# csyxwei/FFWM

Measured on AMD Instinct MI355X. Metric: train img/s (128x128, full FFWM GAN step), higher is better.
Workload: dtype f32; 1 GPU; BASELINE configs[2]: full FFWM train step (netG+netD+flowNetF+flowNetB, all losses, 3x Adam), synthetic MultiPIE-shaped 128x128; batch_per_gpu=8, global_batch=8, parallelism=dp1, grad_buckets=10, bucket_MiB=64

## Files before the change

ffwm_amd/_lib.py:

```python
import ctypes
import os

_HERE = os.path.dirname(os.path.abspath(__file__))
LIB_PATH = os.path.join(_HERE, "lib", "libffwm_hip.so")

F32, F64 = 0, 1
ABI_VERSION = 5

_lib = None

_p = ctypes.c_void_p
_i64 = ctypes.c_int64
_i = ctypes.c_int

_SIGNATURES = {
    "ffwm_block_extractor_forward": [_p, _p, _p] + [_i64] * 6 + [_i, _i, _p],
    "ffwm_block_extractor_backward": [_p, _p, _p, _p, _p] + [_i64] * 6 + [_i, _i, _p],
    "ffwm_block_extractor_backward_strided": [_p, _p, _p, ctypes.POINTER(_i64), _p, _p] + [_i64] * 6 + [_i, _i, _p],
    "ffwm_local_attn_reshape_backward_strided": [_p, ctypes.POINTER(_i64), _p] + [_i64] * 3 + [_i, _i, _i, _p],
    "ffwm_resample2d_backward_strided": [_p, _p, _p, ctypes.POINTER(_i64), _p, _p] + [_i64] * 6 + [_i, _i, _i, _i, _p],
    "ffwm_bn_lrelu_forward": [_p] * 9 + [_i64] * 3 + [ctypes.c_double] * 3 + [_i, _p],
    "ffwm_bn_lrelu_backward": [_p] * 10 + [_i64] * 3 + [ctypes.c_double] + [_i, _p],
    "ffwm_bn_res_act_forward": [_p] * 11 + [_i64] * 3 + [ctypes.c_double] * 3 + [_i, _i, _p],
    "ffwm_bn_res_act_backward": [_p] * 11 + [_i64] * 3 + [ctypes.c_double] + [_i, _i, _p],
    "ffwm_mfm_forward": [_p, _p, _p] + [_i64] * 3 + [_i, _p],
    "ffwm_mfm_backward": [_p, _p, _p, _p] + [_i64] * 3 + [_i, _p],
    "ffwm_add_act_forward": [_p, _p, _p, _i64, _i, ctypes.c_double, _i, _p],
    "ffwm_add_act_backward": [_p, _p, _p, _i64, _i, ctypes.c_double, _i, _p],
    "ffwm_sigmoid_gate_forward": [_p, _p, _p, _p, _p, _i64, _i, _p],
    "ffwm_sigmoid_gate_backward": [_p, _p, _p, _p, _p, _i64, _i, _p],
    "ffwm_bias_relu_forward": [_p, _p, _p] + [_i64] * 3 + [_i, _p],
    "ffwm_bias_act_forward": [_p, _p, _p, _p] + [_i64] * 5 + [_i, ctypes.c_double, _i, _p],
    "ffwm_flow_head_forward": [_p, _p, _p, _p] + [_i64] * 4 + [_i, _p],
    "ffwm_conv_thin_forward": [_p, _p, _p, _p] + [_i64] * 5 + [_i, ctypes.c_double, _i, _p],
    "ffwm_flow_up_forward": [_p, _p, _p, _p] + [_i64] * 4 + [_i, _p],
    "ffwm_shuffle_bias_act_forward": [_p, _p, _p] + [_i64] * 5 + [ctypes.c_double, _i, _p],
    "ffwm_image_head_forward": [_p, _p, _p, _p] + [_i64] * 5 + [_i, _p],
    "ffwm_upsample2x_bilinear_forward": [_p, _p] + [_i64] * 5 + [_i, _p],
    "ffwm_sigmoid_gate_forward_strided": [_p, _p, _p, _p, _p] + [_i64] * 4 + [_i, _p],
    "ffwm_flow_head_backward": [_p, _p, _p, _p, _p] + [_i64] * 4 + [_i, _p],
    "ffwm_flow_up_backward": [_p, _p, _p] + [_i64] * 4 + [_i, _p],
    "ffwm_conv2d_forward": [_p, _p, _p, _p, _p] + [_i64] * 5 + [_i, _i, _i, _i, _i64, _i64, _i, ctypes.c_double, _p, _i64, _i, _p],
    "ffwm_conv2d_wgrad": [_p, _p, _p] + [_i64] * 7 + [_i, _i, _i, _i, _p],
    "ffwm_conv2d_wgrad_tiled": [_p, _p, _p, _p] + [_i64] * 7 + [_i, _i, _i, _i, _i, _p],
    "ffwm_conv3x3_winograd_forward": [_p, _p, _p, _p, _p] + [_i64] * 5 + [_i, _i, ctypes.c_double, _i, _p],
    "ffwm_adam_step": [_p, _p, _p, _p, _i64] + [ctypes.c_double] * 4 + [_i64, _i, _p],
    "ffwm_adam_step_device": [_p, _p, _p, _p, _i64] + [ctypes.c_double] * 4 + [_p, _i, _p],
    "ffwm_sgd_step": [_p, _p, _p, _i64, _p, _p, _i, _p, _p, _i, ctypes.c_double, _i, _p],
    "ffwm_softmax_xent": [_p] * 8 + [_i64, _i64, _i, _p],
    "ffwm_softmax_xent_chunk": [],
    "ffwm_conv3x3_wgrad": [_p, _p, _p, _p] + [_i64] * 5 + [_i, _p],
    "ffwm_conv3x3_wgrad_block": [_p, _p, _p, _p] + [_i64] * 9 + [_i, _p],
    "ffwm_block_attention_forward": [_p, _p, _p, _p] + [_i64] * 6 + [_i, _i, _p],
    "ffwm_block_attention_backward": [_p, _p, _p, _p, _p, _p, _p] + [_i64] * 6 + [_i, _i, _p],
    "ffwm_local_attn_reshape_forward": [_p, _p] + [_i64] * 3 + [_i, _i, _p],
    "ffwm_local_attn_reshape_backward": [_p, _p] + [_i64] * 3 + [_i, _i, _i, _p],
    "ffwm_resample2d_forward": [_p, _p, _p] + [_i64] * 6 + [_i, _i, _i, _p],
    "ffwm_resample2d_backward": [_p, _p, _p, _p, _p] + [_i64] * 6 + [_i, _i, _i, _i, _p],
    "ffwm_warp_forward": [_p, _p, _p] + [_i64] * 6 + [_i, _i, _p],
    "ffwm_warp_backward": [_p, _p, _p, _p, _p] + [_i64] * 6 + [_i, _i, _p],
    "ffwm_warp_multi_forward": [_p, _i, _i, _i, _p],
    "ffwm_warp_multi_backward": [_p, _i, _i, _i, _p],
    "ffwm_spectral_norm_forward": [_p, _i, _i, ctypes.c_double, _i, _p],
    "ffwm_spectral_norm_backward": [_p, _i, _i, _p],
    "ffwm_guided_filter_forward": [_p, _p, _p, _p, _i64, _i64, _i64, _i, ctypes.c_double, _i, _p],
    "ffwm_affine_regularization": [_p, _p, _p, _p, _i64, _i64, _i64, _i, ctypes.c_double, _i, _p],
    "ffwm_correlation_colmax": [_p, _p, _p, _i64, _i64, _i64, _i, _p],
    "ffwm_correlation_colmax_split": [_p, _p, _p, _i64, _i64, _i64, _i, _p],
    "ffwm_sampling_correctness": [_p] * 9 + [_i64] * 6 + [ctypes.c_double, ctypes.c_double, _i, _p],
    "ffwm_landmark_loss": [_p, _p, ctypes.POINTER(_i64), ctypes.POINTER(_i64), ctypes.POINTER(ctypes.c_double), _i] + [_p] * 6
                          + [_i64, _i64, _i, _p],
    "ffwm_guided_filter_backward": [_p, _p, _p, _p, _p, _p, _i64, _i64, _i64, _i, _i, _p],
    "ffwm_guided_filter_forward_general": [_p, _p, _p, _p, _p, _i64, _i64, _i64, _i64, _i, ctypes.c_double, _i, _p],
    "ffwm_guided_filter_backward_general": [_p, _p, _p, _p, _p, _p, _p, _i64, _i64, _i64, _i64, _i, _i, _p],
    "ffwm_l1_multi": [_p, _i, _p, _p, _i, _i, _p],
    "ffwm_conv3x3_winograd_weights_multi": [_p, _i, _i, _p],
    "ffwm_conv3x3_wg_weights": [_p, _p, _i64, _i64, _i, _i, _p],
    "ffwm_conv3x3_wg_forward": [_p, _p, _p, _p, _p] + [_i64] * 5 + [_i, _p, _i, _p],
    "ffwm_conv3x3_wg_forward_tiled": [_p, _p, _p, _p, _p] + [_i64] * 5 + [_i, _p, _i, _i, _p],
    "ffwm_conv3x3_wg_tile": [_i64] * 5,
    "ffwm_mfm_tail_forward": [_p, _p, _p, _p] + [_i64] * 4 + [_i, _i, _p],
    "ffwm_identity_input": [_p, _p] + [_i64] * 4 + [_i, _i, _p],
    "ffwm_identity_input_backward": [_p, _p] + [_i64] * 4 + [_i, _i, _p],
    "ffwm_cosine_topk": [_p, _p, _p, _p] + [_i64] * 4 + [_p, _i64, _i, _p],
    "ffwm_face_batch": [_p] * 16 + [_i64] * 8 + [_i, _p],
    "ffwm_face_gallery": [_p, _p, _p] + [_i64] * 4 + [_p],
    "ffwm_identity_batch": [_p] * 8 + [_i64] * 5 + [_i, _i, _p],
    "ffwm_prof_enable": [_i],
    "ffwm_prof_collect": [],
    "ffwm_prof_get": [_i, ctypes.c_char_p, _i, ctypes.POINTER(_i64), ctypes.POINTER(ctypes.c_double),
                      ctypes.POINTER(ctypes.c_double)],
    "ffwm_prof_get_flops": [_i, ctypes.POINTER(ctypes.c_double)],
    "ffwm_prof_get_bound": [_i, ctypes.POINTER(ctypes.c_double)],
    "ffwm_prof_reset": [],
    "ffwm_set_option": [ctypes.c_char_p, _i],
    "ffwm_zero_fill": [_p, _i64, _p],
    "ffwm_abi_version": [],
}

EXPORTS = sorted(list(_SIGNATURES) + ["ffwm_last_error", "ffwm_conv3x3_winograd_workspace_bytes", "ffwm_conv3x3_winograd_splits",
                                      "ffwm_conv2d_forward_workspace", "ffwm_guided_filter_workspace_bytes",
                                      "ffwm_sampling_correctness_workspace_bytes", "ffwm_landmark_loss_workspace_bytes",
                                      "ffwm_cosine_topk_workspace_bytes", "ffwm_softmax_xent_workspace_bytes",
                                      "ffwm_conv3x3_wg_weights_bytes", "ffwm_conv3x3_wg_workspace_bytes"])


class FFWMError(RuntimeError):
    pass


def load():
    global _lib
    if _lib is not None:
        return _lib
    if not os.path.exists(LIB_PATH):
        raise FFWMError(
            "libffwm_hip.so is missing (%s). The HIP extension is the only implementation of the "
            "ffwm_amd ops -- build it with `python -m ffwm_amd.build`." % LIB_PATH)
    lib = ctypes.CDLL(LIB_PATH)
    for name, argtypes in _SIGNATURES.items():
        fn = getattr(lib, name)
        fn.argtypes = argtypes
        fn.restype = _i
    lib.ffwm_conv3x3_winograd_workspace_bytes.argtypes = [_i64, _i64]
    lib.ffwm_conv3x3_winograd_workspace_bytes.restype = _i64
    lib.ffwm_conv3x3_winograd_splits.argtypes = [_i64, _i64, _i64, _i64, _i64, _i]
    lib.ffwm_conv3x3_winograd_splits.restype = _i
# ... 71 lines not shown
```

ffwm_amd/conv.py:

```python
import os as _os

import torch
import torch.nn as nn
from torch.autograd import Function

from . import ops

_WGRAD_W64 = _os.environ.get("FFWM_WGRAD_W64", "1") == "1"


class _Conv3x3MfmaWgrad(Function):

    @staticmethod
    def forward(ctx, x, weight, bias):
        ctx.save_for_backward(x, weight)
        ctx.has_bias = bias is not None
        return torch.ops.aten.convolution(x, weight, bias, [1, 1], [1, 1], [1, 1], False, [0, 0], 1)

    @staticmethod
    @torch.autograd.function.once_differentiable
    def backward(ctx, grad_output):
        x, weight = ctx.saved_tensors
        go = grad_output.contiguous()
        need_x, need_w, need_b = ctx.needs_input_grad[0], ctx.needs_input_grad[1], ctx.has_bias and ctx.needs_input_grad[2]
# ... 27 lines not shown
                and input.is_cuda and input.dtype == torch.float32 and not torch.is_autocast_enabled()):
            return _MfmaConv2d.apply(input, weight, bias, self.stride[0], self.padding[0], False)
        return super()._conv_forward(input, weight, bias)


def _tiled_wgrad_layer_ok(m):
    if m.kernel_size == (1, 1):
        return (_TILED_WGRAD and _TILED_WGRAD_1X1 and m.stride == (1, 1) and m.padding == (0, 0) and m.dilation == (1, 1) and m.groups == 1
                and min(m.in_channels, m.out_channels) >= 32)
    return (_TILED_WGRAD and m.kernel_size in ((3, 3), (4, 4)) and m.stride in ((1, 1), (2, 2)) and m.padding[0] == m.padding[1]
            and m.padding[0] < m.kernel_size[0] and m.dilation == (1, 1) and m.groups == 1 and m.padding_mode == "zeros")


def eligible(m):
    return (type(m) is nn.Conv2d and m.kernel_size == (3, 3) and m.stride == (1, 1) and m.padding == (1, 1)
            and m.dilation == (1, 1) and m.groups == 1 and m.padding_mode == "zeros"
            and (min(m.in_channels, m.out_channels) >= 64
                 or (min(m.in_channels, m.out_channels) <= 3 and max(m.in_channels, m.out_channels) >= 64)))


def route_conv_wgrad(net):
    n = 0
    for m in net.modules():
        if eligible(m):
            m.__class__ = MfmaWgradConv2d
            n += 1
    return n


_TILED_WGRAD = _os.environ.get("FFWM_TILED_WGRAD", "1") != "0"
_TILED_WGRAD_1X1 = _os.environ.get("FFWM_TILED_WGRAD_1X1", "1") != "0"


def _tiled_wgrad_wins(rows, gathered, kernel):
    K, P = rows.shape[1], rows.shape[2] * rows.shape[3]
    if not (_TILED_WGRAD and kernel in (1, 3, 4) and ops.conv2d_wgrad_tiled_ok(rows) and gathered.numel() < (1 << 29)):
        return False
    if kernel == 1 and (min(K, gathered.shape[1]) < 32 or not _TILED_WGRAD_1X1):
        return False
    if K <= 4 and (P >= 16384 or (P >= 4096 and gathered.shape[1] >= 128)):
        return False
    return True


class _GradArena:

    def __init__(self):
        self.buf, self.off, self.need, self.active, self.retired = None, 0, 0, False, []

    def begin(self, device):
        self.off = self.need = 0
        if self.buf is not None and self.buf.device != device:
            self.retired.append(self.buf)
            self.buf = None
        if self.buf is not None:
            ops.zero_fill(self.buf)
        self.active = True
        self.device = device

    def take(self, n, like):
        if not self.active or like.device != self.device or like.dtype != torch.float32:
            return None
        n_al = (n + 63) & ~63
        self.need += n_al
        if self.buf is None or self.off + n_al > self.buf.numel():
            return None
        s = self.buf[self.off:self.off + n]
        self.off += n_al
        return s

    def end(self):
        if not self.active:
            return
        self.active = False
        if (self.buf is None or self.need > self.buf.numel()) and self.need > 0 and not torch.cuda.is_current_stream_capturing():
            if self.buf is not None:
                self.retired.append(self.buf)
            self.buf = torch.zeros(self.need + self.need // 8, device=self.device, dtype=torch.float32)


GRAD_ARENA = _GradArena()


def conv_weight_grad(x, go, weight, stride, pad, need_b):
    k = weight.shape[2]
    if k == 3 and stride == 1 and pad == 1 and wgrad_route_ok(x, weight):
        n = weight.numel()
        total = n + (weight.shape[0] if need_b else 0)
        buf = GRAD_ARENA.take(total, go)
        if buf is None:
            buf = torch.zeros(total, device=go.device, dtype=go.dtype)
        gw, gb = buf[:n].view_as(weight), (buf[n:] if need_b else None)
        ops.conv3x3_wgrad(x, go, gw, gb)
        return gw, gb
    if _tiled_wgrad_wins(go, x, k) and weight.shape[2] == weight.shape[3]:
        return ops.conv2d_wgrad_tiled(go, x, k, stride, pad, want_bias=bool(need_b),
                                      zeroed=GRAD_ARENA.take(weight.numel() + (weight.shape[0] if need_b else 0), go))
    _, gw, gb = torch.ops.aten.convolution_backward(go, x, weight, [weight.shape[0]] if need_b else None, [stride, stride], [pad, pad],
                                                    [1, 1], False, [0, 0], 1, [False, True, bool(need_b)])
    return gw, gb


def conv_transpose_weight_grad(x, go, weight, need_b):
    if _tiled_wgrad_wins(x, go, 4):
        gw, _ = ops.conv2d_wgrad_tiled(x, go, 4, 2, 1, zeroed=GRAD_ARENA.take(weight.numel(), go))
        return gw, (_bias_grad(go) if need_b else None)
    _, gw, gb = torch.ops.aten.convolution_backward(go, x, weight, [weight.shape[1]] if need_b else None, [2, 2], [1, 1], [1, 1], True,
                                                    [0, 0], 1, [False, True, bool(need_b)])
    return gw, gb


_WINOGRAD = _os.environ.get("FFWM_WINOGRAD", "1") != "0"
WINOGRAD_MIN_TILES = int(_os.environ.get("FFWM_WINOGRAD_MIN_TILES", 2048))
WINOGRAD_MIN_PAIRS = int(_os.environ.get("FFWM_WINOGRAD_MIN_PAIRS", 160))


def _winograd_dir_ok(x, c_red, k_out, act=0):
    tiles = x.shape[0] * ((x.shape[2] + 1) // 2) * ((x.shape[3] + 1) // 2)
    if not (min(c_red, k_out) >= 32 and tiles >= WINOGRAD_MIN_TILES and x.shape[0] * max(c_red, k_out) * x.shape[2] * x.shape[3] < (1 << 29)):
        return False
    pairs = ((tiles + 63) // 64) * ((k_out + 63) // 64)
    if pairs < WINOGRAD_MIN_PAIRS and act == 0:
        pairs *= ops.conv3x3_winograd_splits(x.shape[0], c_red, x.shape[2], x.shape[3], k_out, act)
    return pairs >= WINOGRAD_MIN_PAIRS


def winograd_dirs(x, weight, act=0):
    if not (_WINOGRAD and x.is_cuda and x.dtype == torch.float32 and weight.dtype == torch.float32 and x.dim() == 4
            and not torch.is_autocast_enabled()):
        return False, False
    K, C = weight.shape[0], weight.shape[1]
    if K <= 4 and C >= 32:
        return x.shape[3] % 4 == 0 and x.shape[0] * x.shape[2] * x.shape[3] >= 65536 and x.numel() < (1 << 29), False
    return _winograd_dir_ok(x, C, K, act), _winograd_dir_ok(x, K, C)


def winograd_ok(x, weight, act=0):
    return winograd_dirs(x, weight, act)[0]


_WINO_BATCH = _os.environ.get("FFWM_WINO_BATCH", "1") != "0"


def _note_winograd_use(weight, x, dirs, need_dgrad):
    owner = getattr(weight, "_ffwm_wino_owner", None)
    if owner is None or not _WINO_BATCH:
        return None
    keys = owner.__dict__.setdefault("_wino_keys", set())
    wm4 = x.shape[3] % 4 == 0
    if dirs[0]:
        keys.add((0, wm4))
    if dirs[1] and need_dgrad:
        keys.add((1, wm4))
    return getattr(weight, "_ffwm_wino", None)


class _WinogradConv3x3(Function):

    @staticmethod
    def forward(ctx, x, weight, bias, frozen=None, dirs=(True, True)):
        pre = _note_winograd_use(weight, x, dirs, ctx.needs_input_grad[0])
        x, weight = x.contiguous(), weight.contiguous()
        ctx.save_for_backward(x, weight)
        ctx.has_bias = bias is not None
        ctx.frozen = frozen
        ctx.own_dgrad = dirs[1]
        ctx.wino_pre = pre
        if dirs[0]:
            return ops.conv3x3_winograd(x, weight, bias, frozen=frozen, pre=pre)
        return torch.ops.aten.convolution(x, weight, bias, [1, 1], [1, 1], [1, 1], False, [0, 0], 1)

    @staticmethod
    @torch.autograd.function.once_differentiable
    def backward(ctx, grad_output):
        x, weight = ctx.saved_tensors
        go = grad_output.contiguous()
        need_x, need_w, need_b = ctx.needs_input_grad[0], ctx.needs_input_grad[1], ctx.has_bias and ctx.needs_input_grad[2]
        gx = gw = gb = None
        if need_x and ctx.own_dgrad:
            gx = ops.conv3x3_winograd(go, weight, None, data_gradient=True, frozen=ctx.frozen, pre=ctx.wino_pre)
        elif need_x:
            gx = torch.ops.aten.convolution_backward(go, x, weight, None, [1, 1], [1, 1], [1, 1], False, [0, 0], 1, [True, False, False])[0]
        if need_w:
            gw, gb = conv_weight_grad(x, go, weight, 1, 1, need_b)
        if need_b and gb is None:
            gb = _bias_grad(go)
# ... 485 lines not shown
```

ffwm_amd/ops.py:

```python
import ctypes

import torch

from . import _lib

_DT = {torch.float32: _lib.F32, torch.float64: _lib.F64}


def _dtype_code(t):
    try:
        return _DT[t.dtype]
    except KeyError:
        raise TypeError("ffwm_amd ops support float32/float64 (AT_DISPATCH_FLOATING_TYPES), got %s" % t.dtype)


def _go_strides(grad_output):
    if grad_output.is_contiguous():
        return grad_output, None
    st = grad_output.stride()
    if any(x < 0 for x in st) or st[3] == 0:
        return grad_output.contiguous(), None
    return grad_output, (ctypes.c_int64 * 4)(*st)


# ... 559 lines not shown
                                         _ptr(ws), B, N, code, stream), "ffwm_softmax_xent")
    return out, row_loss, rank, grad, skipped


def conv3x3_wgrad_supported(input, grad_output):
    return (input.dtype == torch.float32 and grad_output.dtype == torch.float32 and input.is_cuda
            and input.shape[3] % 64 == 0 and input.numel() * 4 < (1 << 32) - 64 and grad_output.numel() * 4 < (1 << 32) - 64)


def conv3x3_wgrad(input, grad_output, grad_weight=None, grad_bias=None):
    _check("conv3x3_wgrad", input, grad_output, grad_weight)
    if grad_bias is not None and not (grad_bias.is_cuda and grad_bias.device == input.device and grad_bias.dtype == input.dtype
                                      and grad_bias.is_contiguous()):
        raise ValueError("conv3x3_wgrad: grad_bias must be a contiguous tensor on the input's device, same dtype")
    B, C, H, W = input.shape
    Bg, K, Hg, Wg = grad_output.shape
    if (Bg, Hg, Wg) != (B, H, W):
        raise ValueError("conv3x3_wgrad: grad_output %s does not match input %s" % (tuple(grad_output.shape), tuple(input.shape)))
    if grad_weight is None:
        grad_weight = input.new_zeros((K, C, 3, 3))
    elif tuple(grad_weight.shape) != (K, C, 3, 3):
        raise ValueError("conv3x3_wgrad: grad_weight has the wrong shape")
    if grad_bias is not None and tuple(grad_bias.shape) != (K,):
        raise ValueError("conv3x3_wgrad: grad_bias has the wrong shape")
    with _on_device(input) as stream:
        _lib.check(_lib.load().ffwm_conv3x3_wgrad(_ptr(input), _ptr(grad_output), _ptr(grad_weight), _ptr(grad_bias), B, C, K,
                                                  H, W, _dtype_code(input), stream), "ffwm_conv3x3_wgrad")
    return grad_weight


def conv2d_wgrad(rows, gathered, kernel, stride, pad, grad_weight=None):
    _check("conv2d_wgrad", rows, gathered, grad_weight)
    B, K, Ho, Wo = rows.shape
    Bg, C, H, W = gathered.shape
    if Bg != B:
        raise ValueError("conv2d_wgrad: batch sizes differ")
    if grad_weight is None:
        grad_weight = rows.new_zeros((K, C, kernel, kernel))
    elif tuple(grad_weight.shape) != (K, C, kernel, kernel):
        raise ValueError("conv2d_wgrad: grad_weight has the wrong shape")
    with _on_device(rows) as stream:
        _lib.check(_lib.load().ffwm_conv2d_wgrad(_ptr(rows), _ptr(gathered), _ptr(grad_weight), B, K, Ho, Wo, C, H, W, int(kernel),
                                                 int(stride), int(pad), _dtype_code(rows), stream), "ffwm_conv2d_wgrad")
    return grad_weight


def zero_fill(t):
    if not (t.is_cuda and t.is_contiguous()):
        raise ValueError("zero_fill: a contiguous CUDA tensor")
    with _on_device(t) as stream:
        _lib.check(_lib.load().ffwm_zero_fill(_ptr(t), t.numel() * t.element_size(), stream), "ffwm_zero_fill")
    return t


def conv2d_wgrad_tiled_ok(rows):
    return (rows.is_cuda and rows.dtype == torch.float32 and rows.dim() == 4 and (rows.shape[2] * rows.shape[3]) % 4 == 0
            and rows.data_ptr() % 16 == 0 and rows.numel() < (1 << 29))


def conv2d_wgrad_tiled(rows, gathered, kernel, stride, pad, want_bias=False, zeroed=None):
    _check("conv2d_wgrad_tiled", rows, gathered)
    B, K, Ho, Wo = rows.shape
    Bg, C, H, W = gathered.shape
    if Bg != B:
        raise ValueError("conv2d_wgrad_tiled: batch sizes differ")
    n = K * C * kernel * kernel
    total = n + (K if want_bias else 0)
    if zeroed is not None:
        if not (zeroed.is_cuda and zeroed.device == rows.device and zeroed.dtype == rows.dtype and zeroed.is_contiguous() and zeroed.numel() == total):
            raise ValueError("conv2d_wgrad_tiled: `zeroed` must be %d contiguous zero elements of the operands' device and dtype" % total)
        buf = zeroed.view(-1)
    else:
        buf = rows.new_empty((total,))
    gw = buf[:n].view(K, C, kernel, kernel)
    gb = buf[n:] if want_bias else None
    lib = _lib.load()
    with _on_device(rows) as stream:
        _lib.check(lib.ffwm_conv2d_wgrad_tiled(_ptr(rows), _ptr(gathered), _ptr(gw), _ptr(gb), B, K, Ho, Wo, C, H, W, int(kernel),
                                               int(stride), int(pad), 1 if zeroed is not None else 0, _dtype_code(rows), stream),
                   "ffwm_conv2d_wgrad_tiled")
    return gw, gb


def conv3x3_winograd(x, weight, bias=None, data_gradient=False, act=0, slope=0.0, out=None, frozen=None, pre=None):
    _check("conv3x3_winograd", x, weight, out)
    if bias is not None and (not bias.is_cuda or bias.dtype != x.dtype or not bias.is_contiguous()):
        raise ValueError("conv3x3_winograd: bias must be a contiguous tensor of the input's device and dtype")
    B, C, H, W = x.shape
    if data_gradient:
        if weight.shape[0] != C or tuple(weight.shape[2:]) != (3, 3):
            raise ValueError("conv3x3_winograd: weight %s does not belong to a grad_output with %d channels" % (tuple(weight.shape), C))
        K = weight.shape[1]
    else:
        if weight.shape[1] != C or tuple(weight.shape[2:]) != (3, 3):
            raise ValueError("conv3x3_winograd: weight %s does not fit an input with %d channels" % (tuple(weight.shape), C))
        K = weight.shape[0]
    if bias is not None and tuple(bias.shape) != (K,):
        raise ValueError("conv3x3_winograd: bias must have %d elements" % K)
    if out is None:
        out = x.new_empty((B, K, H, W))
    elif tuple(out.shape) != (B, K, H, W):
        raise ValueError("conv3x3_winograd: out has the wrong shape")
    lib = _lib.load()
    _sync_winograd_split_mode()
    mode = int(bool(data_gradient))
    ws = None
    if pre is not None:
        ws = pre.get((mode, W % 4 == 0))
        if ws is not None:
            mode |= 2
            frozen = None
    if ws is None and frozen is not None and frozen is not False:
        key = (mode, W % 4 == 0, weight._version, weight.data_ptr())
        ws = frozen.get(key)
        if ws is not None:
            mode |= 2
        else:
            for k in [k for k in frozen if k[2:] != key[2:]]:
                del frozen[k]
    if ws is None:
        ws = x.new_empty((lib.ffwm_conv3x3_winograd_workspace_bytes(K, C) // 4,))
        if frozen is not None and frozen is not False:
            frozen[key] = ws
    with _on_device(x) as stream:
        _lib.check(lib.ffwm_conv3x3_winograd_forward(_ptr(x), _ptr(weight), _ptr(bias) if bias is not None else None, _ptr(out), _ptr(ws),
                                                     B, C, H, W, K, mode, int(act), float(slope), _dtype_code(x),
                                                     stream), "ffwm_conv3x3_winograd_forward")
    if frozen is not None and frozen is not False and not (mode & 2):
        torch.cuda.current_stream(x.device).synchronize()
    return out


class _WinoWeightsItem(ctypes.Structure):
    _fields_ = [("weight", ctypes.c_void_p), ("workspace", ctypes.c_void_p), ("K", ctypes.c_int64), ("C", ctypes.c_int64),
                ("data_gradient", ctypes.c_int), ("width_multiple_of_4", ctypes.c_int)]


def conv3x3_winograd_weights_multi(items):
    if not items:
        return []
    lib = _lib.load()
    w0 = items[0][0]
    arr = (_WinoWeightsItem * len(items))()
    out = []
    for a, (w, dg, wm4) in zip(arr, items):
        if not (w.is_cuda and w.dtype == torch.float32 and w.is_contiguous() and w.dim() == 4 and tuple(w.shape[2:]) == (3, 3) and w.device == w0.device):
            raise ValueError("conv3x3_winograd_weights_multi: contiguous float32 [K, C, 3, 3] weights on one GPU")
        K, C = (w.shape[1], w.shape[0]) if dg else (w.shape[0], w.shape[1])
        ws = w.new_empty((lib.ffwm_conv3x3_winograd_workspace_bytes(K, C) // 4,))
        a.weight, a.workspace, a.K, a.C, a.data_gradient, a.width_multiple_of_4 = w.data_ptr(), ws.data_ptr(), K, C, int(bool(dg)), int(bool(wm4))
        out.append(ws)
    with _on_device(w0) as stream:
        _lib.check(lib.ffwm_conv3x3_winograd_weights_multi(ctypes.cast(arr, ctypes.c_void_p), len(items), _lib.F32, stream),
                   "ffwm_conv3x3_winograd_weights_multi")
    return out


_WINO_SPLIT_CAPPED = False
_WINO_SPLIT_BEFORE_CAP = 1


def _sync_winograd_split_mode():
    global _WINO_SPLIT_CAPPED, _WINO_SPLIT_BEFORE_CAP
    want = bool(torch.are_deterministic_algorithms_enabled())
    if want == _WINO_SPLIT_CAPPED:
        return
# ... 474 lines not shown
```

include/ffwm_hip.h:

```cpp
#ifndef FFWM_HIP_H_
#define FFWM_HIP_H_

#include <stdint.h>

#ifdef __cplusplus
extern "C" {
#endif

#define FFWM_ABI_VERSION 5

typedef enum {
    FFWM_OK = 0,
    FFWM_ERR_ARG = -1,
    FFWM_ERR_DTYPE = -2,
    FFWM_ERR_SIZE = -3,
    FFWM_ERR_LAUNCH = -4
} ffwm_status;

typedef enum { FFWM_F32 = 0, FFWM_F64 = 1 } ffwm_dtype;

int ffwm_abi_version(void);
const char* ffwm_last_error(void);

int ffwm_block_extractor_forward(const void* source, const void* flow_field, void* output,
// ... 130 lines not shown

int64_t ffwm_landmark_loss_workspace_bytes(const int64_t* sides, int n_scales, int64_t B, int64_t L, int dtype);
int ffwm_landmark_loss(const void* const* flows, void* const* grads, const int64_t* sides, const int64_t* divisors,
                       const double* weights, int n_scales, const void* lm_S, const void* lm_F, const void* gate,
                       void* out, void* skipped, void* workspace, int64_t B, int64_t L, int dtype, void* stream);

int ffwm_block_attention_forward(const void* source, const void* flow_field, const void* weights, void* output,
                                 int64_t B, int64_t C, int64_t Hs, int64_t Ws, int64_t Hf, int64_t Wf,
                                 int kernel_size, int dtype, void* stream);

int ffwm_block_attention_backward(const void* source, const void* flow_field, const void* weights,
                                  const void* grad_output, void* grad_source, void* grad_flow_field,
                                  void* grad_weights, int64_t B, int64_t C, int64_t Hs, int64_t Ws, int64_t Hf,
                                  int64_t Wf, int kernel_size, int dtype, void* stream);

int ffwm_conv3x3_wgrad(const void* input, const void* grad_output, void* grad_weight, void* grad_bias, int64_t B,
                       int64_t C, int64_t K, int64_t H, int64_t W, int dtype, void* stream);

int ffwm_conv3x3_wgrad_block(const void* input, const void* grad_output, void* grad_weight, void* grad_bias, int64_t B,
                             int64_t C, int64_t K, int64_t H, int64_t W, int64_t k_begin, int64_t k_end, int64_t c_begin,
                             int64_t c_end, int dtype, void* stream);

int ffwm_bn_lrelu_forward(const void* x, const void* weight, const void* bias, void* running_mean, void* running_var,
                          void* y, void* save_mean, void* save_invstd, void* scratch, int64_t B, int64_t C, int64_t HW,
                          double eps, double momentum, double negative_slope, int dtype, void* stream);

int ffwm_bn_lrelu_backward(const void* x, const void* grad_out, const void* weight, const void* bias,
                           const void* save_mean, const void* save_invstd, void* grad_x, void* grad_weight,
                           void* grad_bias, void* scratch, int64_t B, int64_t C, int64_t HW, double negative_slope,
                           int dtype, void* stream);

int ffwm_bn_res_act_forward(const void* x, const void* weight, const void* bias, void* running_mean, void* running_var,
                            const void* res, const void* rbias, void* y, void* save_mean, void* save_invstd, void* scratch,
                            int64_t B, int64_t C, int64_t HW, double eps, double momentum, double negative_slope, int act,
                            int dtype, void* stream);
int ffwm_bn_res_act_backward(const void* x, const void* y, const void* grad_out, const void* weight, const void* save_mean,
                             const void* save_invstd, void* grad_x, void* grad_res, void* grad_weight, void* grad_bias,
                             void* scratch, int64_t B, int64_t C, int64_t HW, double negative_slope, int act, int dtype,
                             void* stream);

int ffwm_mfm_forward(const void* x, const void* bias, void* y, int64_t B, int64_t C, int64_t HW, int dtype, void* stream);
int ffwm_mfm_backward(const void* x, const void* bias, const void* grad_y, void* grad_x, int64_t B, int64_t C, int64_t HW,
                      int dtype, void* stream);

int ffwm_add_act_forward(const void* a, const void* b, void* y, int64_t n, int act, double negative_slope, int dtype, void* stream);
int ffwm_add_act_backward(const void* y, const void* grad_y, void* grad_z, int64_t n, int act, double negative_slope, int dtype,
                          void* stream);
int ffwm_sigmoid_gate_forward(const void* a, const void* b, const void* x, void* att, void* y, int64_t n, int dtype, void* stream);
int ffwm_sigmoid_gate_backward(const void* x, const void* att, const void* grad_y, void* grad_z, void* grad_x, int64_t n, int dtype,
                               void* stream);

int ffwm_bias_relu_forward(const void* h, const void* bias, void* y, int64_t B, int64_t C, int64_t HW, int dtype, void* stream);

int ffwm_bias_act_forward(const void* h, const void* bias, void* y, void* y2, int64_t B, int64_t C, int64_t HW,
                          int64_t y_batch_stride, int64_t y2_batch_stride, int act, double negative_slope, int dtype,
                          void* stream);
int ffwm_conv_thin_forward(const void* x, const void* weight_ctk, const void* bias, void* y, int64_t B, int64_t C, int64_t H, int64_t W,
                           int64_t K, int act, double negative_slope, int dtype, void* stream);

int ffwm_flow_head_forward(const void* x, const void* weight, const void* bias, void* y, int64_t B, int64_t C, int64_t H,
                           int64_t W, int dtype, void* stream);
int ffwm_flow_up_forward(const void* flow, const void* weight, const void* bias, void* out, int64_t B, int64_t H, int64_t W,
                         int64_t out_batch_stride, int dtype, void* stream);

int ffwm_flow_head_backward(const void* y, const void* grad_y, const void* weight, void* grad_z, void* grad_x, int64_t B, int64_t C,
                            int64_t H, int64_t W, int dtype, void* stream);
int ffwm_flow_up_backward(const void* grad_out, const void* weight, void* grad_x, int64_t B, int64_t H, int64_t W,
                          int64_t grad_out_batch_stride, int dtype, void* stream);

int64_t ffwm_conv2d_forward_workspace(int64_t B, int64_t C, int64_t H, int64_t W, int64_t K, int kernel, int stride, int pad,
                                      int transposed);
int ffwm_conv2d_forward(const void* input, const void* weight, const void* bias, void* output, void* output2, int64_t B, int64_t C,
                        int64_t H, int64_t W, int64_t K, int kernel, int stride, int pad, int transposed, int64_t out_batch_stride,
                        int64_t out2_batch_stride, int act, double negative_slope, void* workspace, int64_t workspace_bytes,
                        int dtype, void* stream);

int ffwm_conv2d_wgrad(const void* rows, const void* gathered, void* grad_weight, int64_t B, int64_t K, int64_t Ho, int64_t Wo,
                      int64_t C, int64_t H, int64_t W, int kernel, int stride, int pad, int dtype, void* stream);

int ffwm_conv2d_wgrad_tiled(const void* rows, const void* gathered, void* grad_weight, void* grad_bias, int64_t B, int64_t K,
                            int64_t Ho, int64_t Wo, int64_t C, int64_t H, int64_t W, int kernel, int stride, int pad, int prezeroed,
                            int dtype, void* stream);

int64_t ffwm_conv3x3_winograd_workspace_bytes(int64_t K, int64_t C);
int ffwm_conv3x3_winograd_splits(int64_t B, int64_t C, int64_t H, int64_t W, int64_t K, int act);

typedef struct ffwm_wino_weights {
    const void* weight;
    void* workspace;
    int64_t K, C;
    int data_gradient;
    int width_multiple_of_4;
} ffwm_wino_weights;
int ffwm_conv3x3_winograd_weights_multi(const ffwm_wino_weights* items, int n, int dtype, void* stream);
int ffwm_conv3x3_winograd_forward(const void* input, const void* weight, const void* bias, void* output, void* workspace,
                                  int64_t B, int64_t C, int64_t H, int64_t W, int64_t K, int data_gradient, int act,
                                  double slope, int dtype, void* stream);

enum { FFWM_WG_NONE = 0, FFWM_WG_BIAS = 1, FFWM_WG_BIAS_RELU = 2, FFWM_WG_BIAS_MFM = 3 };
int64_t ffwm_conv3x3_wg_weights_bytes(int64_t K, int64_t C);
int64_t ffwm_conv3x3_wg_workspace_bytes(int64_t B, int64_t C, int64_t H, int64_t W, int64_t K);
int ffwm_conv3x3_wg_weights(const void* weight, void* U, int64_t K, int64_t C, int data_gradient, int dtype, void* stream);
int ffwm_conv3x3_wg_forward(const void* input, const void* U, const void* bias, void* output, void* workspace,
                            int64_t B, int64_t C, int64_t H, int64_t W, int64_t K, int epilogue, const void* relu_mask,
                            int dtype, void* stream);
int ffwm_conv3x3_wg_tile(int64_t B, int64_t C, int64_t H, int64_t W, int64_t K);
int ffwm_conv3x3_wg_forward_tiled(const void* input, const void* U, const void* bias, void* output, void* workspace,
                                  int64_t B, int64_t C, int64_t H, int64_t W, int64_t K, int epilogue, const void* relu_mask,
                                  int tile, int dtype, void* stream);

int ffwm_adam_step(void* params, const void* grads, void* exp_avg, void* exp_avg_sq, int64_t n, double lr,
                   double beta1, double beta2, double eps, int64_t step, int dtype, void* stream);

int ffwm_adam_step_device(void* params, const void* grads, void* exp_avg, void* exp_avg_sq, int64_t n, double lr, double beta1,
                          double beta2, double eps, void* state, int dtype, void* stream);

int ffwm_sgd_step(void* params, const void* grads, void* momentum_buf, int64_t n, const int64_t* seg_end, const int32_t* seg_group,
                  int n_seg, const double* group_lr, const double* group_wd, int n_groups, double momentum, int dtype, void* stream);

int ffwm_softmax_xent_chunk(void);
int64_t ffwm_softmax_xent_workspace_bytes(int64_t B, int64_t N, int dtype);
int ffwm_softmax_xent(const void* logits, const int64_t* target, void* out, void* row_loss, int* rank, void* grad_logits,
                      int* skipped, void* workspace, int64_t B, int64_t N, int dtype, void* stream);

int ffwm_shuffle_bias_act_forward(const void* h, const void* bias, void* y, int64_t B, int64_t K, int64_t H, int64_t W,
                                  int64_t y_batch_stride, double negative_slope, int dtype, void* stream);
int ffwm_image_head_forward(const void* x, const void* weight, const void* bias, void* y, int64_t B, int64_t C, int64_t H, int64_t W,
                            int64_t y_batch_stride, int dtype, void* stream);
int ffwm_upsample2x_bilinear_forward(const void* x, void* y, int64_t B, int64_t C, int64_t H, int64_t W, int64_t y_batch_stride,
                                     int dtype, void* stream);
int ffwm_sigmoid_gate_forward_strided(const void* a, const void* b, const void* x, void* att, void* y, int64_t B, int64_t C,
                                      int64_t HW, int64_t y_batch_stride, int dtype, void* stream);

int ffwm_mfm_tail_forward(const void* h, const void* bias, const void* residual, void* y, int64_t B, int64_t C, int64_t H, int64_t W,
                          int pool, int dtype, void* stream);
int ffwm_identity_input(const void* img, void* out, int64_t B, int64_t Cin, int64_t H, int64_t W, int crop, int dtype, void* stream);
int ffwm_identity_input_backward(const void* grad_out, void* grad_img, int64_t B, int64_t Cin, int64_t H, int64_t W, int crop, int dtype,
                                 void* stream);
int64_t ffwm_cosine_topk_workspace_bytes(int64_t B, int64_t G, int64_t D, int64_t k);
int ffwm_cosine_topk(const void* probe, const void* gallery, void* values, void* indices, int64_t B, int64_t G, int64_t D, int64_t k,
                     void* workspace, int64_t workspace_bytes, int dtype, void* stream);

int ffwm_face_batch(const void* images, const void* masks, const void* pairs, const void* pair_lm, const void* lm, const void* lm_flip,
                    const void* gate, const void* index, void* img_S, void* img_F, void* mask_S, void* mask_F, void* lm_S, void* lm_F,
                    void* gate_out, void* invalid, int64_t N, int64_t H, int64_t W, int64_t P, int64_t K, int64_t KG, int64_t L,
                    int64_t B, int train, void* stream);
int ffwm_face_gallery(const void* images, const void* rows, void* out, int64_t N, int64_t H, int64_t W, int64_t G, void* stream);
int ffwm_identity_batch(const void* images, const void* targets, const void* index, const void* matrix, const void* flip, void* img,
                        void* target, void* invalid, int64_t N, int64_t H, int64_t W, int64_t B, int64_t out_side, int augment,
                        int crop, void* stream);

int ffwm_prof_enable(int on);
int ffwm_prof_collect(void);
int ffwm_prof_get(int row, char* name, int name_len, int64_t* launches, double* total_ms,
                  double* algorithmic_bytes);
int ffwm_prof_get_flops(int row, double* algorithmic_flops);
int ffwm_prof_get_bound(int row, double* roofline_ms);
int ffwm_prof_reset(void);

int ffwm_set_option(const char* key, int value);

int ffwm_zero_fill(void* p, int64_t bytes, void* stream);

#ifdef __cplusplus
}
#endif
// ... 2 lines not shown
```

Baseline: 218.6 img/s.

## Add MFMA stream weight-gradient kernel for small-pixel convolutions

Adds a HIP kernel that computes convolution weight gradients for layers with few output pixels (at most 512 batch-by-plane pixels) as one pass over pixel chunks. Each workgroup owns a 64x64 tile of output channels by input taps, stages rows and gathered im2col columns in LDS, and accumulates with fp32 MFMA. Bias gradients are fused in. A per-shape table routes specific deep-layer shapes (512-1026 channels, 3x3 and transposed 4x4) to it. The aim is to cut launch and split-K overhead of the existing wgrad paths on tiny spatial sizes, at the cost of a low-parallelism serial reduction over pixels per tile.

Measured after the change: 221.3 img/s (median of 6 runs). No clear change (+1.2%).

```diff
diff --git a/ffwm_amd/_lib.py b/ffwm_amd/_lib.py
--- a/ffwm_amd/_lib.py
+++ b/ffwm_amd/_lib.py
@@ -5,6 +5,7 @@
 LIB_PATH = os.path.join(_HERE, "lib", "libffwm_hip.so")
 
 F32, F64 = 0, 1
+STREAM_WGRAD = 2
 ABI_VERSION = 5
 
 _lib = None
@@ -43,6 +44,8 @@
     "ffwm_conv2d_forward": [_p, _p, _p, _p, _p] + [_i64] * 5 + [_i, _i, _i, _i, _i64, _i64, _i, ctypes.c_double, _p, _i64, _i, _p],
     "ffwm_conv2d_wgrad": [_p, _p, _p] + [_i64] * 7 + [_i, _i, _i, _i, _p],
     "ffwm_conv2d_wgrad_tiled": [_p, _p, _p, _p] + [_i64] * 7 + [_i, _i, _i, _i, _i, _p],
+    "ffwm_conv2d_stream_wgrad": [_p, _p, _p, _p] + [_i64] * 7 + [_i, _i, _i, _i, _i, _p],
+    "ffwm_conv2d_stream_plan": [_i] + [_i64] * 5 + [_i, _i, _i, _i, ctypes.POINTER(_i64)],
     "ffwm_conv3x3_winograd_forward": [_p, _p, _p, _p, _p] + [_i64] * 5 + [_i, _i, ctypes.c_double, _i, _p],
     "ffwm_adam_step": [_p, _p, _p, _p, _i64] + [ctypes.c_double] * 4 + [_i64, _i, _p],
     "ffwm_adam_step_device": [_p, _p, _p, _p, _i64] + [ctypes.c_double] * 4 + [_p, _i, _p],
diff --git a/ffwm_amd/conv.py b/ffwm_amd/conv.py
--- a/ffwm_amd/conv.py
+++ b/ffwm_amd/conv.py
@@ -133,8 +133,34 @@
 GRAD_ARENA = _GradArena()
 
 
+_STREAM = _os.environ.get("FFWM_CONV_STREAM", "1") != "0"
+_ST_NEVER = (1, 0)
+STREAM_TABLE = {
+    (512, 512, 3, 1, False): {"wgrad": (64, 512)},
+    (512, 512, 3, 2, False): {"wgrad": (64, 128)},
+    (512, 1024, 3, 2, False): {"wgrad": (16, 32)},
+    (1024, 1024, 3, 1, False): {"wgrad": (16, 32)},
+    (1024, 512, 4, 2, True): {"wgrad": (16, 32)},
+    (1026, 512, 3, 1, False): {"wgrad": (64, 128)},
+    (1026, 256, 4, 2, True): {"wgrad": (64, 128)},
+    (770, 256, 3, 1, False): {"wgrad": (512, 512)},
+    (770, 128, 4, 2, True): {"wgrad": (256, 512)},
+}
+
+
+def stream_route(direction, C, K, kernel, stride, transposed, n):
+    if not _STREAM or n > ops.STREAM_MAX_PIXELS:
+        return False
+    lo, hi = STREAM_TABLE.get((C, K, kernel, stride, bool(transposed)), {}).get(direction, _ST_NEVER)
+    return lo <= n <= hi
+
+
 def conv_weight_grad(x, go, weight, stride, pad, need_b):
     k = weight.shape[2]
+    if (stream_route("wgrad", weight.shape[1], weight.shape[0], k, stride, False, go.shape[0] * go.shape[2] * go.shape[3])
+            and weight.shape[2] == weight.shape[3] and not torch.is_autocast_enabled() and ops.conv2d_stream_wgrad_ok(go, x, k, stride, pad)):
+        return ops.conv2d_stream_wgrad(go, x, k, stride, pad, want_bias=bool(need_b),
+                                       out=GRAD_ARENA.take(weight.numel() + (weight.shape[0] if need_b else 0), go))
     if k == 3 and stride == 1 and pad == 1 and wgrad_route_ok(x, weight):
         n = weight.numel()
         total = n + (weight.shape[0] if need_b else 0)
@@ -153,6 +179,10 @@
 
 
 def conv_transpose_weight_grad(x, go, weight, need_b):
+    if (stream_route("wgrad", weight.shape[0], weight.shape[1], 4, 2, True, x.shape[0] * x.shape[2] * x.shape[3])
+            and not torch.is_autocast_enabled() and ops.conv2d_stream_wgrad_ok(x, go, 4, 2, 1)):
+        return ops.conv2d_stream_wgrad(x, go, 4, 2, 1, want_bias=bool(need_b), bias_of_gathered=True,
+                                       out=GRAD_ARENA.take(weight.numel() + (weight.shape[1] if need_b else 0), go))
     if _tiled_wgrad_wins(x, go, 4):
         gw, _ = ops.conv2d_wgrad_tiled(x, go, 4, 2, 1, zeroed=GRAD_ARENA.take(weight.numel(), go))
         return gw, (_bias_grad(go) if need_b else None)
diff --git a/ffwm_amd/csrc/conv_stream.hip b/ffwm_amd/csrc/conv_stream.hip
--- /dev/null
+++ b/ffwm_amd/csrc/conv_stream.hip
@@ -0,0 +1,301 @@
+#include "common.hpp"
+
+namespace ffwm {
+namespace {
+
+typedef float f32x16 __attribute__((ext_vector_type(16)));
+typedef float f32x4 __attribute__((ext_vector_type(4)));
+
+constexpr int kSwMaxPixels = 512;
+constexpr int kSwPC = 32;
+constexpr int kSwP = 36;
+constexpr int kSwDepth = 1;
+constexpr int kSwT = 64;
+constexpr int64_t kSwMaxGrid = 1 << 20;
+
+struct SwGeo {
+    int C, H, W, K, Ho, Wo, stride, pad;
+    int N, P, HW;
+    int total_px;
+    int chunks;
+    int bias_mode;
+    unsigned a_bytes, x_bytes;
+    FastDiv divP, divWo;
+};
+
+template <int R, int S>
+__global__ void __launch_bounds__(kBlock, 4)
+conv_stream_wgrad_kernel(const float* __restrict__ a, const float* __restrict__ x, float* __restrict__ dw, float* __restrict__ gbias,
+                         const SwGeo g) {
+    constexpr int RS = R * S;
+    constexpr int TM = kSwT, TN = kSwT;
+    constexpr int NQA = TM * 8 / kBlock;
+    constexpr int NXB = TN / 8;
+    constexpr int D = kSwDepth;
+    extern __shared__ __attribute__((aligned(16))) unsigned char smem_raw[];
+    float* lds = reinterpret_cast<float*>(smem_raw);
+    const int lane = threadIdx.x & 63, wave = threadIdx.x >> 6;
+    const int l31 = lane & 31, half = lane >> 5;
+    const int wm = wave >> 1, wn = wave & 1;
+    const int n0 = blockIdx.x * TN, k0 = blockIdx.y * TM;
+    constexpr unsigned kOobOff = 0xFFFFFFF0u;
+    const rsrc_t ra_ = make_rsrc(a, g.a_bytes);
+    const rsrc_t rx_ = make_rsrc(x, g.x_bytes);
+
+    const int q8 = threadIdx.x & 7, arow0 = threadIdx.x >> 3;
+    unsigned arow_off[NQA];
+#pragma unroll
+    for (int i = 0; i < NQA; ++i) {
+        const int k = k0 + arow0 + 32 * i;
+        arow_off[i] = k < g.K ? static_cast<unsigned>(k) * static_cast<unsigned>(g.P) : kOobOff;
+    }
+    const int kk = threadIdx.x & 31, xcol0 = threadIdx.x >> 5;
+    int coloff[NXB];
+    unsigned colsh[NXB];
+#pragma unroll
+    for (int i = 0; i < NXB; ++i) {
+        const int n = n0 + xcol0 + 8 * i;
+        const bool cin = n < g.N;
+        const int nc = cin ? n : 0;
+        const int c = nc / RS, rs = nc - c * RS;
+        const int r = rs / S, sx = rs - r * S;
+        coloff[i] = c * g.HW + r * g.W + sx;
+        colsh[i] = cin ? static_cast<unsigned>(8 * r + sx) : 31u;
+    }
+
+    const bool bias_rows = g.bias_mode == 1 && blockIdx.x == 0;
+    const bool bias_cols = g.bias_mode == 2 && blockIdx.y == 0;
+
+    f32x4 va[D][NQA];
+    float vx[D][NXB];
+    float bsum[NQA], xsum[NXB];
+#pragma unroll
+    for (int i = 0; i < NQA; ++i) bsum[i] = 0.f;
+#pragma unroll
+    for (int i = 0; i < NXB; ++i) xsum[i] = 0.f;
+
+    auto fetch = [&](int ch, f32x4 (&ra)[NQA], float (&rb)[NXB]) {
+        {
+            const unsigned gq = static_cast<unsigned>(ch) * kSwPC + q8 * 4;
+            const unsigned b = fast_div(gq, g.divP);
+            const unsigned p = gq - b * static_cast<unsigned>(g.P);
+            const unsigned a_pin = 0u - static_cast<unsigned>(gq < static_cast<unsigned>(g.total_px));
+            const unsigned a_base = b * static_cast<unsigned>(g.K) * static_cast<unsigned>(g.P) + p;
+#pragma unroll
+            for (int i = 0; i < NQA; ++i) {
+                const unsigned live = a_pin & (0u - static_cast<unsigned>(arow_off[i] != kOobOff));
+                const unsigned off = (((a_base + arow_off[i]) * 4u) & live) | (kOobOff & ~live);
+                const u32x4 v = __builtin_amdgcn_raw_buffer_load_b128(ra_, off, 0, 0);
+                ra[i][0] = __uint_as_float(v.x); ra[i][1] = __uint_as_float(v.y); ra[i][2] = __uint_as_float(v.z); ra[i][3] = __uint_as_float(v.w);
+            }
+        }
+        {
+            const unsigned gq = static_cast<unsigned>(ch) * kSwPC + kk;
+            const unsigned b = fast_div(gq, g.divP);
+            const unsigned p = gq - b * static_cast<unsigned>(g.P);
+            const unsigned pin = static_cast<unsigned>(gq < static_cast<unsigned>(g.total_px));
+            const int oy = static_cast<int>(fast_div(p, g.divWo)), ox = static_cast<int>(p) - oy * g.Wo;
+            const int iy0 = oy * g.stride - g.pad, ix0 = ox * g.stride - g.pad;
+            unsigned rmask = 0, smask = 0;
+#pragma unroll
+            for (int r = 0; r < R; ++r) rmask |= static_cast<unsigned>(static_cast<unsigned>(iy0 + r) < static_cast<unsigned>(g.H)) << r;
+#pragma unroll
+            for (int q = 0; q < S; ++q) smask |= static_cast<unsigned>(static_cast<unsigned>(ix0 + q) < static_cast<unsigned>(g.W)) << q;
+            unsigned taps = 0;
+#pragma unroll
+            for (int r = 0; r < R; ++r) taps |= (smask & (0u - ((rmask >> r) & 1u))) << (8 * r);
+            const int x_inv = static_cast<int>(~(taps & (0u - pin)));
+            const int x_base = static_cast<int>(b) * g.C * g.HW + iy0 * g.W + ix0;
+#pragma unroll
+            for (int i = 0; i < NXB; ++i) {
+                const unsigned dead = static_cast<unsigned>(__builtin_amdgcn_sbfe(x_inv, colsh[i], 1u));
+                rb[i] = buf_ld<float>(rx_, (static_cast<unsigned>(x_base + coloff[i]) << 2) | dead);
+            }
+        }
+    };
+    auto commit = [&](int buf, const f32x4 (&ra)[NQA], const float (&rb)[NXB]) {
+        float* As = lds + buf * (TM + TN) * kSwP;
+        float* Xs = As + TM * kSwP;
+#pragma unroll
+        for (int i = 0; i < NQA; ++i) {
+            *reinterpret_cast<f32x4*>(As + (arow0 + 32 * i) * kSwP + q8 * 4) = ra[i];
+            if (bias_rows) bsum[i] += (ra[i][0] + ra[i][1]) + (ra[i][2] + ra[i][3]);
+        }
+#pragma unroll
+        for (int i = 0; i < NXB; ++i) {
+            Xs[(xcol0 + 8 * i) * kSwP + kk] = rb[i];
+            if (bias_cols) xsum[i] += rb[i];
+        }
+    };
+
+    f32x16 acc;
+#pragma unroll
+    for (int r = 0; r < 16; ++r) acc[r] = 0.f;
+
+    auto compute = [&](int buf) {
+        const float* As = lds + buf * (TM + TN) * kSwP;
+        const float* Xs = As + TM * kSwP;
+        const float* ap = As + (wm * 32 + l31) * kSwP + 4 * half;
+        const float* bp = Xs + (wn * 32 + l31) * kSwP + 4 * half;
+#pragma unroll
+        for (int gq = 0; gq < kSwPC / 8; ++gq) {
+            const f32x4 av = *reinterpret_cast<const f32x4*>(ap + 8 * gq);
+            const f32x4 bv = *reinterpret_cast<const f32x4*>(bp + 8 * gq);
+#pragma unroll
+            for (int q = 0; q < 4; ++q) acc = __builtin_amdgcn_mfma_f32_32x32x2f32(av[q], bv[q], acc, 0, 0, 0);
+        }
+    };
+
+#pragma unroll
+    for (int s = 0; s < D; ++s)
+        if (s < g.chunks) fetch(s, va[s], vx[s]);
+    for (int base = 0; base < g.chunks; base += D) {
+#pragma unroll
+        for (int s = 0; s < D; ++s) {
+            const int ch = base + s;
+            if (ch < g.chunks) {
+                commit(ch & 1, va[s], vx[s]);
+                if (ch + D < g.chunks) fetch(ch + D, va[s], vx[s]);
+                __syncthreads();
+                compute(ch & 1);
+            }
+        }
+    }
+
+    const int n = n0 + wn * 32 + l31;
+    if (n < g.N) {
+#pragma unroll
+        for (int r = 0; r < 16; ++r) {
+            const int k = k0 + wm * 32 + (r & 3) + 8 * (r >> 2) + 4 * half;
+            if (k < g.K) dw[static_cast<size_t>(k) * g.N + n] = acc[r];
+        }
+    }
+    if (bias_rows) {
+#pragma unroll
+        for (int i = 0; i < NQA; ++i) {
+            float v = bsum[i];
+            v += __shfl_xor(v, 1, 64);
+            v += __shfl_xor(v, 2, 64);
+            v += __shfl_xor(v, 4, 64);
+            const int k = k0 + arow0 + 32 * i;
+            if (q8 == 0 && k < g.K) gbias[k] = v;
+        }
+    }
+    if (bias_cols) {
+        __syncthreads();
+#pragma unroll
+        for (int i = 0; i < NXB; ++i) {
+            float v = xsum[i];
+#pragma unroll
+            for (int o = 1; o < 32; o <<= 1) v += __shfl_xor(v, o, 64);
+            if (kk == 0) lds[xcol0 + 8 * i] = v;
+        }
+        __syncthreads();
+        const int t = threadIdx.x;
+        if (t < TN / RS && n0 + RS * t < g.N) {
+            const float* cs = lds + RS * t;
+            gbias[(n0 + RS * t) / RS] = (cs[S + 1] + cs[S + 2]) + (cs[2 * S + 1] + cs[2 * S + 2]);
+        }
+    }
+}
+
+}
+}
+
+using namespace ffwm;
+
+namespace {
+
+struct SwPlan {
+    int k_tiles = 0, n_tiles = 0;
+};
+
+int sw_geometry(const char* fn, int64_t B, int64_t K, int64_t Ho, int64_t Wo, int64_t C, int64_t H, int64_t W, int kernel, int stride,
+                int pad, int bias_mode, SwGeo* g, SwPlan* p) {
+    FFWM_REQUIRE(B > 0 && K > 0 && C > 0 && Ho > 0 && Wo > 0 && H > 0 && W > 0, FFWM_ERR_ARG, "%s: sizes must be positive", fn);
+    FFWM_REQUIRE(((kernel == 3 && (stride == 1 || stride == 2)) || (kernel == 4 && stride == 2)) && pad == 1, FFWM_ERR_ARG,
+                 "%s: 3x3 / stride 1 or 2 / pad 1 and 4x4 / stride 2 / pad 1 only (got kernel %d, stride %d, pad %d)", fn, kernel, stride, pad);
+    FFWM_REQUIRE(Ho == (H + 2 * pad - kernel) / stride + 1 && Wo == (W + 2 * pad - kernel) / stride + 1, FFWM_ERR_ARG,
+                 "%s: the row tensor's plane (%lld x %lld) is not the output plane of this convolution over %lld x %lld", fn,
+                 (long long)Ho, (long long)Wo, (long long)H, (long long)W);
+    FFWM_REQUIRE(B * Ho * Wo <= kSwMaxPixels, FFWM_ERR_ARG, "%s: at most %d pixels (batch x row-tensor plane), got %lld", fn, kSwMaxPixels,
+                 (long long)(B * Ho * Wo));
+    FFWM_REQUIRE((Ho * Wo) % 4 == 0, FFWM_ERR_ARG, "%s: the row tensor's plane must hold a multiple of 4 pixels", fn);
+    FFWM_REQUIRE(bias_mode != 2 || (kernel == 4 && H == 2 * Ho && W == 2 * Wo), FFWM_ERR_ARG,
+                 "%s: the bias gradient of the gathered tensor needs a 4x4 kernel over a plane of twice the row tensor's", fn);
+    FFWM_REQUIRE(B * K * Ho * Wo < (1LL << 29) && B * C * H * W < (1LL << 29) && K * C * kernel * kernel < (1LL << 29), FFWM_ERR_SIZE,
+                 "%s: tensors must stay below 2 GiB", fn);
+    g->C = static_cast<int>(C); g->H = static_cast<int>(H); g->W = static_cast<int>(W);
+    g->K = static_cast<int>(K); g->Ho = static_cast<int>(Ho); g->Wo = static_cast<int>(Wo);
+    g->stride = stride; g->pad = pad;
+    g->N = g->C * kernel * kernel;
+    g->P = g->Ho * g->Wo;
+    g->HW = g->H * g->W;
+    g->total_px = static_cast<int>(B) * g->P;
+    g->chunks = (g->total_px + kSwPC - 1) / kSwPC;
+    g->bias_mode = bias_mode;
+    g->a_bytes = static_cast<unsigned>(B * K * Ho * Wo * 4);
+    g->x_bytes = static_cast<unsigned>(B * C * H * W * 4);
+    g->divP = make_fast_div(static_cast<unsigned>(g->P));
+    g->divWo = make_fast_div(static_cast<unsigned>(g->Wo));
+    p->k_tiles = (g->K + kSwT - 1) / kSwT;
+    p->n_tiles = (g->N + kSwT - 1) / kSwT;
+    FFWM_REQUIRE(static_cast<int64_t>(p->k_tiles) * p->n_tiles <= kSwMaxGrid && p->k_tiles <= 65535, FFWM_ERR_SIZE,
+                 "%s: more than %lld workgroups", fn, (long long)kSwMaxGrid);
+    return FFWM_OK;
+}
+
+}
+
+extern "C" int ffwm_conv2d_stream_plan(int pass, int64_t B, int64_t C, int64_t H, int64_t W, int64_t K, int kernel, int stride, int pad,
+                                       int transposed, int64_t* plan) {
+    const char* fn = "ffwm_conv2d_stream_plan";
+    FFWM_REQUIRE(plan != nullptr, FFWM_ERR_ARG, "%s: NULL plan", fn);
+    FFWM_REQUIRE(pass == FFWM_STREAM_WGRAD, FFWM_ERR_ARG, "%s: pass %d is not served (the weight gradient, %d, is)", fn, pass, FFWM_STREAM_WGRAD);
+    FFWM_REQUIRE(transposed == 0 || transposed == 1, FFWM_ERR_ARG, "%s: transposed must be 0 or 1", fn);
+    FFWM_REQUIRE(B > 0 && C > 0 && H > 0 && W > 0 && K > 0 && H < (1 << 20) && W < (1 << 20), FFWM_ERR_ARG, "%s: bad sizes", fn);
+    SwGeo g;
+    SwPlan p;
+    int rc;
+    if (transposed) {
+        FFWM_REQUIRE(kernel == 4 && stride == 2 && pad == 1, FFWM_ERR_ARG, "%s: the transposed convolution is 4x4 / stride 2 / pad 1", fn);
+        rc = sw_geometry(fn, B, C, H, W, K, 2 * H, 2 * W, kernel, stride, pad, 0, &g, &p);
+    } else {
+        FFWM_REQUIRE(kernel >= 1 && kernel <= 16 && (stride == 1 || stride == 2) && pad >= 0 && H + 2 * pad >= kernel && W + 2 * pad >= kernel,
+                     FFWM_ERR_ARG, "%s: bad kernel / stride / pad", fn);
+        rc = sw_geometry(fn, B, K, (H + 2 * pad - kernel) / stride + 1, (W + 2 * pad - kernel) / stride + 1, C, H, W, kernel, stride, pad, 0, &g, &p);
+    }
+    if (rc != FFWM_OK) return rc;
+    plan[0] = 1;
+    plan[1] = g.total_px;
+    plan[2] = static_cast<int64_t>(p.k_tiles) * p.n_tiles;
+    plan[3] = 11;
+    return FFWM_OK;
+}
+
+extern "C" int ffwm_conv2d_stream_wgrad(const void* rows, const void* gathered, void* grad_weight, void* grad_bias, int64_t B, int64_t K,
+                                        int64_t Ho, int64_t Wo, int64_t C, int64_t H, int64_t W, int kernel, int stride, int pad,
+                                        int bias_of_gathered, int dtype, void* stream) {
+    const char* fn = "ffwm_conv2d_stream_wgrad";
+    FFWM_REQUIRE(dtype == FFWM_F32, FFWM_ERR_DTYPE, "%s: float32 only", fn);
+    FFWM_REQUIRE(rows && gathered && grad_weight, FFWM_ERR_ARG, "%s: NULL tensor pointer", fn);
+    SwGeo g;
+    SwPlan p;
+    const int rc = sw_geometry(fn, B, K, Ho, Wo, C, H, W, kernel, stride, pad, grad_bias ? (bias_of_gathered ? 2 : 1) : 0, &g, &p);
+    if (rc != FFWM_OK) return rc;
+    FFWM_REQUIRE((reinterpret_cast<uintptr_t>(rows) & 15) == 0, FFWM_ERR_ARG, "%s: the row tensor must be 16-byte aligned", fn);
+    hipStream_t st = static_cast<hipStream_t>(stream);
+    const double flops = 2.0 * B * g.P * static_cast<double>(g.K) * g.N;
+    const double bytes = 4.0 * (static_cast<double>(B) * K * g.P + static_cast<double>(B) * C * H * W + static_cast<double>(K) * g.N);
+    LaunchScope ls("conv_stream_wgrad", st, bytes, flops);
+    const dim3 grid(static_cast<unsigned>(p.n_tiles), static_cast<unsigned>(p.k_tiles), 1u);
+    const float* a = static_cast<const float*>(rows);
+    const float* x = static_cast<const float*>(gathered);
+    float* dw = static_cast<float*>(grad_weight);
+    float* gb = static_cast<float*>(grad_bias);
+    const bool ok = dispatch<3, 4>(kernel, [&](auto R) {
+        const size_t lds = (g.chunks > 1 ? 2u : 1u) * 2 * kSwT * kSwP * sizeof(float);
+        hipLaunchKernelGGL((conv_stream_wgrad_kernel<R.value, R.value>), grid, dim3(kBlock), lds, st, a, x, dw, gb, g);
+    });
+    return ok ? check_launch(fn) : no_kernel(fn);
+}
diff --git a/ffwm_amd/ops.py b/ffwm_amd/ops.py
--- a/ffwm_amd/ops.py
+++ b/ffwm_amd/ops.py
@@ -665,6 +665,55 @@
     return gw, gb
 
 
+STREAM_MAX_PIXELS = 512
+
+
+def conv2d_stream_plan(direction, B, C, H, W, K, kernel, stride, pad=1, transposed=False):
+    if direction != "wgrad":
+        return None
+    plan = (ctypes.c_int64 * 4)()
+    rc = _lib.load().ffwm_conv2d_stream_plan(_lib.STREAM_WGRAD, int(B), int(C), int(H), int(W), int(K), int(kernel), int(stride), int(pad),
+                                             1 if transposed else 0, plan)
+    if rc != 0:
+        return None
+    return {"slices": int(plan[0]), "terms": int(plan[1]), "grid": int(plan[2]), "tile": (int(plan[3]) // 10 * 64, int(plan[3]) % 10 * 64)}
+
+
+def conv2d_stream_wgrad_ok(rows, gathered, kernel, stride, pad):
+    if not (rows.is_cuda and rows.dtype == torch.float32 and gathered.dtype == torch.float32 and rows.dim() == 4 and gathered.dim() == 4
+            and gathered.device == rows.device):
+        return False
+    B, K, Ho, Wo = rows.shape
+    _, C, H, W = gathered.shape
+    return (pad == 1 and ((kernel == 3 and stride in (1, 2)) or (kernel == 4 and stride == 2)) and gathered.shape[0] == B
+            and Ho == (H + 2 - kernel) // stride + 1 and Wo == (W + 2 - kernel) // stride + 1
+            and 0 < B * Ho * Wo <= STREAM_MAX_PIXELS and (Ho * Wo) % 4 == 0 and rows.data_ptr() % 16 == 0
+            and gathered.numel() < (1 << 29) and K * C * kernel * kernel < (1 << 29))
+
+
+def conv2d_stream_wgrad(rows, gathered, kernel, stride, pad, want_bias=False, bias_of_gathered=False, out=None):
+    _check("conv2d_stream_wgrad", rows, gathered)
+    B, K, Ho, Wo = rows.shape
+    Bg, C, H, W = gathered.shape
+    if Bg != B:
+        raise ValueError("conv2d_stream_wgrad: batch sizes differ")
+    n = K * C * kernel * kernel
+    total = n + ((C if bias_of_gathered else K) if want_bias else 0)
+    if out is not None:
+        if not (out.is_cuda and out.device == rows.device and out.dtype == rows.dtype and out.is_contiguous() and out.numel() == total):
+            raise ValueError("conv2d_stream_wgrad: `out` must be %d contiguous elements of the operands' device and dtype" % total)
+        buf = out.view(-1)
+    else:
+        buf = rows.new_empty((total,))
+    gw = buf[:n].view(K, C, kernel, kernel)
+    gb = buf[n:] if want_bias else None
+    with _on_device(rows) as stream:
+        _lib.check(_lib.load().ffwm_conv2d_stream_wgrad(_ptr(rows), _ptr(gathered), _ptr(gw), _ptr(gb), B, K, Ho, Wo, C, H, W, int(kernel),
+                                                        int(stride), int(pad), 1 if bias_of_gathered else 0, _dtype_code(rows), stream),
+                   "ffwm_conv2d_stream_wgrad")
+    return gw, gb
+
+
 def conv3x3_winograd(x, weight, bias=None, data_gradient=False, act=0, slope=0.0, out=None, frozen=None, pre=None):
     _check("conv3x3_winograd", x, weight, out)
     if bias is not None and (not bias.is_cuda or bias.dtype != x.dtype or not bias.is_contiguous()):
diff --git a/include/ffwm_hip.h b/include/ffwm_hip.h
--- a/include/ffwm_hip.h
+++ b/include/ffwm_hip.h
@@ -236,6 +236,14 @@
                             int64_t Ho, int64_t Wo, int64_t C, int64_t H, int64_t W, int kernel, int stride, int pad, int prezeroed,
                             int dtype, void* stream);
 
+int ffwm_conv2d_stream_wgrad(const void* rows, const void* gathered, void* grad_weight, void* grad_bias, int64_t B, int64_t K,
+                             int64_t Ho, int64_t Wo, int64_t C, int64_t H, int64_t W, int kernel, int stride, int pad,
+                             int bias_of_gathered, int dtype, void* stream);
+
+#define FFWM_STREAM_WGRAD 2
+int ffwm_conv2d_stream_plan(int pass, int64_t B, int64_t C, int64_t H, int64_t W, int64_t K, int kernel, int stride, int pad,
+                            int transposed, int64_t* plan);
+
 int64_t ffwm_conv3x3_winograd_workspace_bytes(int64_t K, int64_t C);
 int ffwm_conv3x3_winograd_splits(int64_t B, int64_t C, int64_t H, int64_t W, int64_t K, int act);
 
```
